# mkkellogg/GaussianSplats3D

Measured on AMD Instinct MI355X. Metric: Msplats/s sorted+rasterized at 1920x1080 SH-2, higher is better.
Workload: dtype int32 keys / f32 raster; 1 GPU; C3: garden.ply stand-in, SH2, 1920x1080; splats=5800000, sh_degree=2, width=1920, height=1080, cull=off (R=N), sort_precision_bits=16, streams=one (SURVEY.md 8d: sort -> draw on a single stream), parallelism=1 GPU, sort=full list (R = N)

## Files before the change

### gaussiansplats3d_amd/csrc/gs_internal.hpp

```cpp
#pragma once
#include <hip/hip_runtime.h>
#include <stdint.h>
#include <stdio.h>
#include <stdlib.h>
#include <string.h>
#include <new>
#include <utility>
#include <vector>

#include "../../include/gsplat_hip.h"
#include "draw_plan.hpp"

void gs_set_error(const char* fmt, ...);

#define GS_HIP(expr)                                                                              \
    do {                                                                                          \
        hipError_t _e = (expr);                                                                   \
        if (_e != hipSuccess) {                                                                   \
            gs_set_error("%s failed: %s (%s:%d)", #expr, hipGetErrorString(_e), __FILE__, __LINE__); \
            return GS_ERR_HIP;                                                                    \
        }                                                                                         \
    } while (0)

#define GS_REQUIRE(cond, msg)                                    \
// ... 162 lines not shown
    __host__ __device__ int32_t hi() const {
        int32_t v = key_max[0];
        for (uint32_t k = 1; k < SORT_SHARDS; k++) v = key_max[k] > v ? key_max[k] : v;
        return v;
    }
    uint32_t clamped;
    uint32_t kept;
};

struct gs_tree;
struct TreeGatherView {
    uint64_t tree_uid;
    uint32_t leaves, tree_splats;
    const uint32_t *leaf_offset, *leaf_count, *leaf_begin, *leaf_indexes, *totals;
};
void gs_tree_view(gs_tree* t, TreeGatherView* v);
int gs_tree_copy_plain(gs_tree* t, uint32_t* out_dev, hipStream_t st);
void gs_tree_forget_sorter(gs_tree* t, gs_sorter* s);

struct AssetDeviceImage {
    DevBuf bytes, table;
};

struct gs_sorter {
    gs_context* ctx = nullptr;
    AssetDeviceImage asset_dev;
    uint32_t max_count = 0, flags = 0, precision = 16, uploaded = 0;
    DevBuf cx, cy, cz, cw, scene_idx;
    DevBuf caos;
    DevBuf staging;
    DevBuf idx_in;
    DevBuf precomputed;
    DevBuf keys;
    DevBuf keyA, keyB, valA, valB;
    DevBuf sorted;
    DevBuf frame;
    uint32_t frame_index = 0;
    DevBuf scene_rows;
    DevBuf debug;
    RadixScratch radix;
    hipStream_t stream = nullptr;
    bool own_stream = false;
    hipEvent_t ev0 = nullptr, ev1 = nullptr;
    bool timed_sort = false;
    hipEvent_t ev_consumed = nullptr;
    bool consumer_pending = false;
    gs_mesh* bound_mesh = nullptr;
    gs_mesh* result_mesh = nullptr;
    const uint32_t* result_unmap = nullptr;
    uint32_t result_payload_max = 0;
    uint32_t gathered = 0;
    bool has_gathered = false;
    bool gathered_on_device = false;
    DevBuf gathered_dev;
    gs_tree* pending_tree = nullptr;
    bool pending_keep_zeroed = false;
    uint32_t centers_version = 0;
    DevBuf pay_in;
    DevBuf leaf_centers, leaf_pos;
    uint64_t leaf_cache_tree = 0;
    uint32_t leaf_cache_centers = 0, leaf_cache_layout = 0, leaf_cache_uploaded = 0;
    const void* leaf_cache_mesh = nullptr;
    uint32_t last_render = 0, last_sort = 0, last_passes = 0;
    bool last_identity = true;
    bool has_result = false;
    bool frustum_cull = false;
    bool visibility_cull = false;
    bool last_culled = false;
    const SortFrame* result_frame = nullptr;
    DevBuf keep_mask;
    DevBuf chunk_counts;
    DevBuf mask_copy;
    bool last_vis_culled = false;
    bool dev_distances = false;
    uint32_t dev_distances_count = 0;
    bool dev_distances_integer = false;
    hipEvent_t ev_handover = nullptr;
    std::vector<int32_t> extreme;
    bool extreme_ok = true;
    uint32_t extreme_version = 0;
    uint32_t clean_slot = 3;
    bool last_known_range = false;
    int32_t last_range_lo = 0, last_range_hi = 0;
    uint32_t last_pass0_slot = 0;
};

struct __attribute__((aligned(32))) SplatRec {
    float cx, cy, ax, ay;
    float bx, by;
    uint32_t c0, c1;
};
static_assert(sizeof(SplatRec) == 32, "SplatRec must be one 32-byte sector");

struct RenderFrame {
    uint32_t visible;
    uint32_t entries_lo;
    uint32_t entries_hi;
    uint32_t overflow;
    uint32_t entry_count;
    uint32_t tiles16_lo;
    uint32_t tiles16_hi;
    uint32_t pad;
};

struct ProjectParams {
    float view[16];
    float proj[16];
    float cam_pos[3];
    float focal_x, focal_y;
    float width, height;
    float splat_scale, kernel2d, max_splat_px, inv_focal_adj;
    uint32_t sh_degree;
    uint32_t sh_stored;
    uint32_t cov_half;
    uint32_t flags;
    uint32_t tiles_x, tiles_y;
    uint32_t row_begin, row_end;
// ... 170 lines not shown
```

### gaussiansplats3d_amd/csrc/sorter.hip

```cpp
#include <math.h>
#include <stdlib.h>

#include "extreme_set.hpp"
#include "radix.hpp"

__host__ __device__ static inline int32_t trunc_f64_i32(double v) {
    if (!(v > -2147483649.0 && v < 2147483648.0)) return INT32_MIN;
    return (int32_t)v;
}

constexpr uint32_t MODE_INT = 1, MODE_DYNAMIC = 2, MODE_PRECOMPUTED = 4;
#ifndef GS_KEY_GRID_MULT
#define GS_KEY_GRID_MULT 2
#endif

struct SceneRows {
    int32_t im[GS_MAX_SCENES][4];
    float fm[GS_MAX_SCENES][4];
};

struct KeyParams {
    const uint32_t *cx, *cy, *cz, *cw;
    const uint4* aos;
    const uint32_t* scene_idx;
// ... 641 lines not shown
        for (uint32_t u = 0; u < VC_UNROLL; u++) {
            const uint32_t i0 = wbase + u * VC_WAVE_SPAN + 4u * lane;
            if (i0 < end && (i0 & 31u) == 0u) {
                mask_copy[i0 >> 5] = cur.raw[u];
                if (cur.raw[u]) mask[i0 >> 5] = 0u;
            }
            uint32_t o = wave_out + first[u];
            const uint32_t pm[4] = {cur.M[u].x, cur.M[u].y, cur.M[u].z, cur.M[u].w};
#pragma unroll
            for (uint32_t c = 0; c < 4u; c++)
                if ((nibs[u] >> c) & 1u) {
                    keys_out[o] = K[u][c];
                    pay_out[o] = pm[c];
                    o++;
                }
        }
        cur = nxt;
    }
    mm.publish_wave(p.frame, blockIdx.x * 4u + wave);
}

struct DepthLoaderArgs {
    const int32_t* __restrict__ keys;
    const unsigned long long* __restrict__ keep;
    const uint32_t* __restrict__ idx;
    const uint32_t* __restrict__ map;
    SortFrame* frame;
    const uint32_t* n_dev;
    uint32_t sort_start, render_count, range;
    uint32_t last_splat;
    uint32_t count_clamps;
    int32_t lo;
    float range_map;
};
template <bool CULL, bool IDX>
struct DepthLoaderT : DepthLoaderArgs {
    __device__ __forceinline__ void prepare() {
        if (n_dev) render_count = *n_dev;
        const uint32_t l = threadIdx.x & (SORT_SHARDS - 1u);
        set_range(frame->key_min[l], frame->key_max[l]);
    }
    __device__ __forceinline__ void set_range(int32_t lo_shard, int32_t hi) {
        lo = lo_shard;
#pragma unroll
        for (int o = SORT_SHARDS / 2; o > 0; o >>= 1) {
            lo = min(lo, __shfl_xor(lo, o, 64));
            hi = max(hi, __shfl_xor(hi, o, 64));
        }
        set_known_range(lo, hi);
        lo = __builtin_amdgcn_readfirstlane(lo);
        range_map = __uint_as_float(__builtin_amdgcn_readfirstlane(__float_as_uint(range_map)));
    }
    __device__ __forceinline__ void set_known_range(int32_t key_lo, int32_t key_hi) {
        lo = key_lo;
        range_map = __fdiv_rn((float)(range - 1), __fsub_rn((float)key_hi, (float)key_lo));
    }
    __device__ __forceinline__ uint32_t count() const { return render_count - sort_start; }
    __device__ __forceinline__ uint32_t bucket(uint32_t i) const { return bucket_of<false>(keys[i]); }
    template <bool COUNT>
    __device__ __forceinline__ uint32_t bucket_of(int32_t depth) const {
        const int32_t diff = (int32_t)((uint32_t)depth - (uint32_t)lo);
        const float f = __fmul_rn((float)diff, range_map);
        const bool fits = f >= -2147483648.0f && f < 2147483648.0f;
        const int32_t b = fits ? (int32_t)f : 0;
        const bool under = b < 0, over = !under && (uint32_t)b >= range;
        if (COUNT && count_clamps && (under || over)) atomicAdd(&frame->clamped, 1u);
        return under ? 0u : (over ? range - 1u : (uint32_t)b);
    }
    __device__ __forceinline__ uint32_t key(uint32_t j) const { return (range - 1) - bucket(render_count - 1 - j); }
    __device__ __forceinline__ uint32_t payload(uint32_t i) const {
        const uint32_t o = IDX ? min(ld32(idx, i), last_splat) : i;
        return map ? ld32(map, o) : o;
    }
    __device__ __forceinline__ uint32_t val(uint32_t j) const { return payload(render_count - 1 - j); }
    struct Raw { int32_t depth; uint32_t payload; };
    static __device__ __forceinline__ int prof_slot(int) { return 0; }
    __device__ __forceinline__ uint32_t pre(uint32_t j) const {
        const uint32_t i = render_count - 1 - j;
        return IDX ? min(ld32(idx, i), last_splat) : i;
    }
    __device__ __forceinline__ Raw fetch(uint32_t j, uint32_t o) const {
        Raw r;
        r.depth = ld32(keys, render_count - 1 - j);
        r.payload = map ? ld32(map, o) : o;
        return r;
    }
    __device__ __forceinline__ void decode(const Raw& r, uint32_t& k, uint32_t& v) const {
        k = (range - 1) - bucket_of<false>(r.depth);
        v = r.payload;
    }
    typedef int32_t HRaw;
    __device__ __forceinline__ HRaw hist_fetch(uint32_t j) const { return ld32(keys, render_count - 1 - j); }
    __device__ __forceinline__ uint32_t hist_key(HRaw depth) const { return (range - 1) - bucket_of<true>(depth); }
    __device__ __forceinline__ bool valid(uint32_t j) const {
        if (!CULL) return true;
        const uint32_t i = render_count - 1 - j;
        return (ld32(keep, i >> 6) >> (i & 63u)) & 1ull;
    }
};
typedef DepthLoaderT<false, false> DepthLoader;

struct PackedLoader {
    const uint32_t* __restrict__ words;
    const uint32_t* __restrict__ n_dev;
    uint32_t n_host, val_bits;
    __device__ __forceinline__ void prepare() {}
    __device__ __forceinline__ uint32_t count() const { return n_dev ? *n_dev : n_host; }
    struct Raw { uint32_t w; };
    __device__ __forceinline__ uint32_t pre(uint32_t) const { return 0u; }
    __device__ __forceinline__ Raw fetch(uint32_t j, uint32_t) const { return Raw{ld32(words, j)}; }
    __device__ __forceinline__ void decode(const Raw& r, uint32_t& k, uint32_t& v) const {
        k = r.w >> val_bits;
        v = r.w & ((1u << val_bits) - 1u);
    }
    __device__ __forceinline__ bool valid(uint32_t) const { return true; }
    static __device__ __forceinline__ int prof_slot(int) { return 1; }
};

__global__ void k_copy_head(const uint32_t* __restrict__ idx, const uint32_t* __restrict__ map, uint32_t* __restrict__ out,
                            uint32_t n, uint32_t last_splat) {
    for (uint32_t i = blockIdx.x * blockDim.x + threadIdx.x; i < n; i += gridDim.x * blockDim.x) {
        const uint32_t o = idx ? min(idx[i], last_splat) : i;
        out[i] = map ? map[o] : o;
    }
}

__global__ void k_unmap(const uint32_t* __restrict__ in, const uint32_t* __restrict__ unmap, uint32_t* __restrict__ out,
                        uint32_t n, uint32_t last) {
    for (uint32_t i = blockIdx.x * blockDim.x + threadIdx.x; i < n; i += gridDim.x * blockDim.x) out[i] = unmap[min(in[i], last)];
}

constexpr uint32_t KEY_HIST_VECS = 3;
__global__ __launch_bounds__(HIST_THREADS) void k_depth_key_hist(KeyParams p, DepthLoader ld, int32_t key_lo, int32_t key_hi, int shift,
                                                                  uint32_t keep_slot, uint32_t* __restrict__ block_hist,
                                                                  uint32_t* __restrict__ group_rows) {
    __shared__ uint32_t s_hist[4][RADIX_BINS];
    const uint32_t tid = threadIdx.x, t = blockIdx.x * HIST_THREADS + tid;
    sort_begin(p, t, gridDim.x * HIST_THREADS, keep_slot);
    if (t < SORT_SHARDS) {
        p.frame->key_min[t] = key_lo;
        p.frame->key_max[t] = key_hi;
    }
    ld.set_known_range(key_lo, key_hi);
    for (uint32_t k = tid; k < 4u * RADIX_BINS; k += HIST_THREADS) (&s_hist[0][0])[k] = 0;
    __syncthreads();
    uint32_t* hist = s_hist[(tid >> 6) & 3u];
    const uint32_t R = p.render_count;
    const RadixChunk ch = radix_chunk(R);
    const uint32_t j0 = min(ch.tile_begin * (uint32_t)RADIX_TILE, R), j1 = min(ch.tile_end * (uint32_t)RADIX_TILE, R);
    const uint32_t p0 = R - j1, p1 = R - j0;
    auto count = [&](int32_t k) { atomicAdd(&hist[(ld.hist_key(k) >> shift) & 255u], 1u); };
    auto scalars = [&](uint32_t begin, uint32_t end) {
        for (uint32_t i = begin + tid; i < end; i += HIST_THREADS) {
            const int32_t k = static_key_int(p, p.cx[i], p.cy[i], p.cz[i]);
            p.keys_out[i] = k;
            count(k);
        }
    };
    const uint32_t a4 = (p0 + 3u) / 4u, b4 = p1 / 4u;
    if (a4 < b4) {
        scalars(p0, a4 * 4u);
        scalars(b4 * 4u, p1);
        const uint4* x4 = reinterpret_cast<const uint4*>(p.cx);
        const uint4* y4 = reinterpret_cast<const uint4*>(p.cy);
        const uint4* z4 = reinterpret_cast<const uint4*>(p.cz);
        int4* o4 = reinterpret_cast<int4*>(p.keys_out);
        for (uint32_t v0 = a4; v0 < b4; v0 += KEY_HIST_VECS * HIST_THREADS) {
            uint4 x[KEY_HIST_VECS], y[KEY_HIST_VECS], z[KEY_HIST_VECS];
#pragma unroll
            for (uint32_t k = 0; k < KEY_HIST_VECS; k++) {
                const uint32_t v = min(v0 + k * HIST_THREADS + tid, b4 - 1u);
                x[k] = x4[v]; y[k] = y4[v]; z[k] = z4[v];
            }
#pragma unroll
            for (uint32_t k = 0; k < KEY_HIST_VECS; k++) {
                const uint32_t v = v0 + k * HIST_THREADS + tid;
                const int4 key = static_key_int4(p, x[k], y[k], z[k]);
                if (v < b4) {
                    o4[v] = key;
                    count(key.x); count(key.y); count(key.z); count(key.w);
                }
            }
        }
    } else {
        scalars(p0, p1);
    }
    __syncthreads();
    if (tid >= RADIX_BINS || ch.tile_begin >= ch.tile_end) return;
    const uint32_t total = s_hist[0][tid] + s_hist[1][tid] + s_hist[2][tid] + s_hist[3][tid];
    block_hist[ch.id * RADIX_BINS + tid] = total;
    if (total) atomicAdd(&group_rows[(ch.id / RADIX_GROUP) * RADIX_BINS + tid], total);
}

__global__ void k_debug_buckets(DepthLoader ld, int32_t* out) {
    ld.prepare();
    for (uint32_t i = ld.sort_start + blockIdx.x * blockDim.x + threadIdx.x; i < ld.render_count;
         i += gridDim.x * blockDim.x)
        out[i] = (int32_t)ld.bucket(i);
}

struct Pass0Args {
    DepthLoaderArgs ld;
    uint32_t Rs, val_bits;
    int shift;
    bool pack, chunked, wide;
    void* kbuf0;
    uint32_t* vo;
    uint32_t* kept_out;
    int slot;
    bool skip_hist;
};
template <bool CULL, bool IDX>
static int depth_pass0(const RadixExec& ex, const Pass0Args& a) {
    typedef DepthLoaderT<CULL, IDX> L;
    const L d = {a.ld};
    L h = d;
    h.count_clamps = 1;
    if (a.pack && a.chunked) return radix_pass_chunk<L, L, true>(ex, h, a.shift, d, a.Rs, a.shift, a.slot, a.vo, a.val_bits, a.kept_out, a.skip_hist);
    if (a.pack) return radix_pass_ex<L, L, uint8_t, false, false, true>(ex, h, a.shift, d, a.Rs, a.shift, a.slot, (uint8_t*)nullptr, a.vo, nullptr, 0u, a.val_bits, a.kept_out, a.skip_hist);
    if (a.wide) return radix_pass_ex<L, L, uint32_t, true, false, false>(ex, h, a.shift, d, a.Rs, a.shift, a.slot, (uint32_t*)a.kbuf0, a.vo, nullptr, 0u, 0u, a.kept_out, a.skip_hist);
    return radix_pass_ex<L, L, uint16_t, true, false, false>(ex, h, a.shift, d, a.Rs, a.shift, a.slot, (uint16_t*)a.kbuf0, a.vo, nullptr, 0u, 0u, a.kept_out, a.skip_hist);
}

static inline uint32_t grid_for(uint32_t n, uint32_t per_block, uint32_t cap) {
    uint32_t g = (n + per_block - 1) / per_block;
    if (g < 1) g = 1;
    return g > cap ? cap : g;
}

#ifdef GS_RADIX_PROFILE
extern "C" int gs_debug_radix_prof(void* dst) {
    return (int)hipMemcpyFromSymbol(dst, HIP_SYMBOL(g_radix_prof), sizeof(g_radix_prof), 0, hipMemcpyDeviceToHost);
}
#endif

extern "C" {

int gs_sorter_create(gs_context* ctx, uint32_t max_splat_count, uint32_t flags, uint32_t precision_bits,
                     gs_sorter** out) {
    GS_REQUIRE(ctx && out, "ctx / out == NULL");
    *out = nullptr;
    GS_REQUIRE(max_splat_count > 0, "max_splat_count == 0");
    GS_REQUIRE((flags & ~(GS_SORT_INTEGER | GS_SORT_DYNAMIC)) == 0, "unknown sorter flags");
    const uint32_t max_bits = (flags & GS_SORT_INTEGER) ? 20u : 24u;
    GS_REQUIRE(precision_bits >= 10 && precision_bits <= max_bits, "precision outside the Viewer's clamp (10..20 int, 10..24 float)");
    ScopedDevice sd(ctx->device);
    gs_sorter* s = new (std::nothrow) gs_sorter();
    if (!s) return GS_ERR_NOMEM;
    s->ctx = ctx;
    s->max_count = max_splat_count;
    s->flags = flags;
    s->precision = precision_bits;
    const size_t n = max_splat_count, b4 = n * 4;
    int st = GS_OK;
    auto A = [&](DevBuf& b, size_t bytes) { if (st == GS_OK) st = b.alloc(bytes); };
    A(s->cx, b4 + 16); A(s->cy, b4 + 16); A(s->cz, b4 + 16); A(s->caos, n * 16);
    if (flags & GS_SORT_DYNAMIC) { A(s->cw, b4); A(s->scene_idx, b4); A(s->scene_rows, sizeof(SceneRows)); }
    A(s->keys, b4); A(s->keyA, b4); A(s->keyB, b4); A(s->valA, b4); A(s->valB, b4); A(s->sorted, b4);
    A(s->frame, 2 * sizeof(SortFrame));
    if (st == GS_OK) st = s->radix.init();
    if (st == GS_OK && (hipEventCreate(&s->ev0) != hipSuccess || hipEventCreate(&s->ev1) != hipSuccess ||
                        hipEventCreateWithFlags(&s->ev_consumed, hipEventDisableTiming) != hipSuccess ||
                        hipEventCreateWithFlags(&s->ev_handover, hipEventDisableTiming) != hipSuccess)) {
        gs_set_error("hipEventCreate failed");
        st = GS_ERR_HIP;
    }
    if (st == GS_OK) {
        SortFrame init[2];
        for (SortFrame& f : init) {
            for (uint32_t k = 0; k < SORT_SHARDS; k++) { f.key_min[k] = KEY_MIN_INIT; f.key_max[k] = KEY_MAX_INIT; }
            f.clamped = f.kept = 0;
        }
        if (hipMemcpy(s->frame.p, init, sizeof(init), hipMemcpyHostToDevice) != hipSuccess ||
            hipMemset(s->radix.digit_total.p, 0, sizeof(uint32_t) * RADIX_TOTAL_WORDS) != hipSuccess) {
            gs_set_error("initialising the sorter scratch failed");
            st = GS_ERR_HIP;
        }
    }
    if (st == GS_OK) {
        if (ctx->serial) {
            s->stream = ctx->stream;
        } else if (hipStreamCreateWithFlags(&s->stream, hipStreamNonBlocking) == hipSuccess) {
            s->own_stream = true;
        } else {
            gs_set_error("hipStreamCreate(sorter) failed");
            st = GS_ERR_HIP;
        }
    }
    if (st != GS_OK) {
        gs_sorter_destroy(s);
        return st;
// ... 22 lines not shown
    static const bool off = getenv("GSPLAT_NO_KNOWN_RANGE") != nullptr;
    return off;
}

static int sorter_update_extreme(gs_sorter* s, uint32_t from, uint32_t end, uint32_t old_uploaded, bool zero_fill) {
    if (s->flags != GS_SORT_INTEGER || known_range_off()) return GS_OK;
    const bool current = s->extreme_ok && s->extreme_version + 1u == s->centers_version;
    const bool append = from >= old_uploaded;
    if (append && !current) {
        s->extreme_ok = false;
        return GS_OK;
    }
    const uint32_t first = append ? old_uploaded : 0u, last = end > old_uploaded ? end : old_uploaded;
    std::vector<int32_t> rows, out;
    try {
        if (zero_fill && append) rows.assign(4, 0);
        else rows.resize((size_t)(last - first) * 4);
    } catch (const std::bad_alloc&) {
        s->extreme_ok = false;
        return GS_OK;
    }
    if (!(zero_fill && append) && last > first) {
        GS_HIP(hipMemcpyAsync(rows.data(), s->caos.as<uint4>() + first, (size_t)(last - first) * 16, hipMemcpyDeviceToHost, s->stream));
        GS_HIP(hipStreamSynchronize(s->stream));
    }
    const bool prior = append && !s->extreme.empty();
    s->extreme_ok = gs_extreme_set(prior ? s->extreme.data() : nullptr, prior ? s->extreme.size() / 4 : 0, rows.data(), rows.size() / 4,
                                   GS_EXTREME_CAP, out);
    s->extreme.swap(out);
    s->extreme_version = s->centers_version;
    return GS_OK;
}

int gs_sorter_upload_centers(gs_sorter* s, uint32_t from, uint32_t count, const void* centers_aos4,
                             const uint32_t* scene_indexes) {
    GS_REQUIRE(s && centers_aos4, "sorter / centers == NULL");
    GS_REQUIRE((uint64_t)from + count <= s->max_count, "range exceeds max_splat_count");
    GS_REQUIRE(!(s->flags & GS_SORT_DYNAMIC) || scene_indexes, "dynamic sorter needs scene_indexes");
    if (count == 0) return GS_OK;
    ScopedDevice sd(s->ctx->device);
    GS_HIP(hipMemcpyAsync(s->caos.as<uint4>() + from, centers_aos4, (size_t)count * 16, hipMemcpyHostToDevice, s->stream));
    return gs_sorter_commit_centers(s, from, count, scene_indexes);
}

}

int gs_sorter_commit_centers(gs_sorter* s, uint32_t from, uint32_t count, const uint32_t* scene_indexes) {
    hipStream_t st = s->stream;
    uint4* aos = s->caos.as<uint4>() + from;
    hipLaunchKernelGGL(k_aos4_to_soa, dim3(grid_for(count, 256, 4096)), dim3(256), 0, st, aos, count,
                       from, s->cx.as<uint32_t>(), s->cy.as<uint32_t>(), s->cz.as<uint32_t>(),
                       (s->flags & GS_SORT_DYNAMIC) ? s->cw.as<uint32_t>() : nullptr);
    GS_HIP(hipGetLastError());
    if (s->flags & GS_SORT_DYNAMIC)
        GS_HIP(hipMemcpyAsync(s->scene_idx.as<uint32_t>() + from, scene_indexes, (size_t)count * 4, hipMemcpyHostToDevice, st));
    GS_HIP(hipStreamSynchronize(st));
    const uint32_t old_uploaded = s->uploaded;
    if (from + count > s->uploaded) s->uploaded = from + count;
    s->centers_version++;
    GS_TRY(sorter_update_extreme(s, from, from + count, old_uploaded, false));
    sorter_tell_mesh(s);
    return GS_OK;
}

extern "C" {

int gs_sorter_set_uploaded_count(gs_sorter* s, uint32_t count) {
    GS_REQUIRE(s != nullptr, "sorter == NULL");
    GS_REQUIRE(count <= s->max_count, "count exceeds max_splat_count");
    if (count <= s->uploaded) return GS_OK;
    ScopedDevice sd(s->ctx->device);
    hipStream_t st = s->stream;
    const size_t from = s->uploaded, n = count - s->uploaded;
    GS_HIP(hipMemsetAsync(s->caos.as<uint4>() + from, 0, n * 16, st));
    DevBuf* planes[] = {&s->cx, &s->cy, &s->cz, &s->cw, &s->scene_idx};
    for (DevBuf* b : planes)
        if (b->p) GS_HIP(hipMemsetAsync(b->as<uint32_t>() + from, 0, n * 4, st));
    GS_HIP(hipStreamSynchronize(st));
    s->uploaded = count;
    s->centers_version++;
    GS_TRY(sorter_update_extreme(s, (uint32_t)from, count, (uint32_t)from, true));
    sorter_tell_mesh(s);
    return GS_OK;
}

static int sorter_collect_stats(gs_sorter* s, gs_sort_stats* stats) {
    SortFrame f;
    GS_HIP(hipMemcpyAsync(&f, s->frame.as<SortFrame>() + s->frame_index, sizeof(f), hipMemcpyDeviceToHost, s->stream));
    GS_HIP(hipStreamSynchronize(s->stream));
    float ms = 0.f;
    if (s->timed_sort) GS_HIP(hipEventElapsedTime(&ms, s->ev0, s->ev1));
    int32_t key_lo = f.lo(), key_hi = f.hi();
    if (s->last_sort == 0) {
        key_lo = KEY_MIN_INIT;
        key_hi = KEY_MAX_INIT;
        f.clamped = 0;
    }
    stats->device_ms = ms;
    stats->key_min = key_lo;
    stats->key_max = key_hi;
    stats->clamped = f.clamped;
    stats->passes = s->last_passes;
    stats->result_count = s->last_culled ? f.kept : s->last_render;
    return f.clamped ? GS_WARN_KEY_CLAMPED : GS_OK;
}

struct SortSwitches {
    bool tree_no_fuse;
    const char* vis_front;
    bool no_pack;
    bool no_chunk;
    bool no_known_range;
};
static SortSwitches sort_switches() {
    static const bool tree_no_fuse = getenv("GSPLAT_TREE_NO_FUSE") != nullptr;
    static const char* vis_front = getenv("GSPLAT_VIS_FRONT");
    static const bool no_pack = getenv("GSPLAT_NO_SORT_PACK") != nullptr;
    static const bool no_chunk = getenv("GSPLAT_NO_SORT_CHUNK") != nullptr;
    return {tree_no_fuse, vis_front, no_pack, no_chunk, known_range_off()};
}

static bool sorter_mesh_alive(const gs_context* ctx, const gs_mesh* m) {
    for (const gs_mesh* l : ctx->live_meshes)
        if (l == m) return m != nullptr;
    return false;
}

struct ChunkGrid { uint32_t grid, len; };
static ChunkGrid chunk_grid(const gs_context* ctx, uint32_t R, uint32_t unit) {
    const uint32_t units = (R + unit - 1u) / unit;
    const uint32_t grid = units < (uint32_t)ctx->cu_count * 2u ? units : (uint32_t)ctx->cu_count * 2u;
    return {grid, ((units + grid - 1u) / grid) * unit};
}

struct SortPlan {
    const float* mvp;
    const uint32_t* indexes_to_sort;
    bool device_list;
    const void* precomputed;
    const float* transforms;
    const uint32_t* list_count_dev;
    uint32_t R, Rs, sort_start;
    bool pre_device, dynamic;
    bool vis_cull;
    bool cull;
    const uint32_t *map, *unmap;
    uint32_t last_splat;
    uint32_t max_payload, val_bits;
    SortSwitches sw;
    const uint32_t* idx_dev;
    bool fused_tree;
    bool vec4;
    bool vis_front;
    bool known_range;
    int32_t range_lo, range_hi;
    uint32_t pass0_slot;
};

struct Pass0Shape { bool pack, chunked; uint32_t grid; };
static Pass0Shape pass0_shape(const gs_sorter* s, const SortPlan& pl) {
    Pass0Shape sh;
    sh.chunked = !pl.sw.no_chunk && pl.val_bits <= 24u && radix_chunk_grid_for(pl.Rs) != 0u;
    sh.pack = s->precision > 8u && !pl.sw.no_pack && (s->precision - 8u) + pl.val_bits <= 32u;
    sh.grid = (sh.pack && sh.chunked) ? radix_chunk_grid_for(pl.Rs) : radix_grid_for(pl.Rs);
    return sh;
}

static bool sort_known_range(const gs_sorter* s, const SortPlan& pl, const KeyParams& kp, int32_t& lo_out, int32_t& hi_out) {
    if (pl.sw.no_known_range || kp.mode != MODE_INT || pl.idx_dev || pl.device_list || pl.fused_tree || pl.vis_cull || pl.cull ||
        pl.list_count_dev || pl.sort_start != 0u || pl.R != s->uploaded || pl.R == 0u)
        return false;
    if (!s->extreme_ok || s->extreme_version != s->centers_version || s->extreme.empty()) return false;
    const int32_t* c = s->extreme.data();
    const size_t n = s->extreme.size() / 4;
    const int64_t a0 = kp.im0, a1 = kp.im1, a2 = kp.im2;
    const int64_t small = (int64_t)1 << 29;
    __int128 lo, hi;
    if (a0 >= -small && a0 <= small && a1 >= -small && a1 <= small && a2 >= -small && a2 <= small) {
        int64_t l = INT64_MAX, h = INT64_MIN;
        for (size_t i = 0; i < n; i++) {
            const int64_t v = a0 * c[4 * i] + a1 * c[4 * i + 1] + a2 * c[4 * i + 2];
            l = v < l ? v : l;
            h = v > h ? v : h;
        }
        lo = l; hi = h;
    } else {
        lo = hi = (__int128)a0 * c[0] + (__int128)a1 * c[1] + (__int128)a2 * c[2];
        for (size_t i = 1; i < n; i++) {
// ... 199 lines not shown
        if (lazy) derive();
        else hipLaunchKernelGGL(k_mask_count, dim3(wg.grid), dim3(VC_THREADS), 0, st, kp, mask, wg.len, counts);
        if (pl.map) hipLaunchKernelGGL(k_cull_front<true>, dim3(wg.grid), dim3(VC_THREADS), 0, st, kp, mask, s->mask_copy.as<uint32_t>(),
                                       counts, wg.len, pl.map, s->pay_in.as<uint32_t>(), lazy ? DERIVE_SUBS : 1u);
        else hipLaunchKernelGGL(k_cull_front<false>, dim3(wg.grid), dim3(VC_THREADS), 0, st, kp, mask, s->mask_copy.as<uint32_t>(),
                                counts, wg.len, pl.map, s->pay_in.as<uint32_t>(), 1u);
    } else {
        const ChunkGrid cg = chunk_grid(ctx, R, VC_SPAN);
        if (!s->pending_tree) s->has_gathered = false;
        GS_TRY(s->chunk_counts.ensure((size_t)std::max(lazy ? dg.grid * DERIVE_SUBS : 0u, cg.grid) * 4));
        counts = s->chunk_counts.as<uint32_t>();
        if (lazy) derive();
        hipLaunchKernelGGL(k_minmax_count, dim3(cg.grid), dim3(VC_THREADS), 0, st, kp, mask, cg.len, counts);
        hipLaunchKernelGGL(k_mask_compact, dim3(cg.grid), dim3(VC_THREADS), 0, st, mask, s->mask_copy.as<uint32_t>(), counts, R, cg.len,
                           s->idx_in.as<uint32_t>(), kp.frame);
    }
    if (R >= mesh->vis_orig_count && (!lazy || mesh->vis_orig_tail_zero)) mesh->vis_orig_dirty = false;
    pl.idx_dev = s->idx_in.as<uint32_t>();
    kp.idx_in = pl.idx_dev;
    kp.count_dev = &kp.frame->kept;
    kp.ext_minmax = 1u;
    if (!pl.vis_front) hipLaunchKernelGGL(k_depth_key<false>, dim3(grid_for(pl.Rs, 256 * 4, (uint32_t)ctx->cu_count * 2)), dim3(256), 0, st, kp);
    return GS_OK;
}

static int launch_front_end(gs_sorter* s, SortPlan& pl, KeyParams& kp) {
    gs_context* ctx = s->ctx;
    hipStream_t st = s->stream;
    const uint32_t cus = (uint32_t)ctx->cu_count;
    pl.vec4 = (kp.mode == MODE_INT) && !pl.idx_dev;
    pl.known_range = sort_known_range(s, pl, kp, pl.range_lo, pl.range_hi);
    pl.pass0_slot = pl.known_range ? s->clean_slot : 0u;
    s->clean_slot = pl.pass0_slot == 3u ? 0u : 3u;
    if (pl.known_range) {
        DepthLoaderArgs hl = {};
        hl.keys = s->keys.as<int32_t>(); hl.frame = kp.frame; hl.sort_start = 0u; hl.render_count = pl.R; hl.range = 1u << s->precision;
        hl.last_splat = kp.last_splat; hl.count_clamps = 1u;
        hipLaunchKernelGGL(k_depth_key_hist, dim3(pass0_shape(s, pl).grid), dim3(HIST_THREADS), 0, st, kp, DepthLoader{hl}, pl.range_lo,
                           pl.range_hi, 0, pl.pass0_slot, s->radix.block_hist.as<uint32_t>(),
                           s->radix.digit_total.as<uint32_t>() + pl.pass0_slot * RADIX_SLOT_WORDS);
    } else if (pl.fused_tree) {
        GS_TRY(launch_tree_front(s, pl, kp));
    } else if (pl.vis_cull) {
        GS_TRY(launch_vis_cull_front(s, pl, kp));
    } else if (pl.cull) {
        if (pl.vec4) hipLaunchKernelGGL(k_depth_key_cull<true>, dim3(grid_for(pl.Rs, 256 * 16, cus * 2)), dim3(256), 0, st, kp);
        else hipLaunchKernelGGL(k_depth_key_cull<false>, dim3(grid_for(pl.Rs, 256 * 4, cus * 4)), dim3(256), 0, st, kp);
    } else if (pl.vec4) {
        hipLaunchKernelGGL(k_depth_key<true>, dim3(grid_for(pl.Rs, 256 * 16, cus * GS_KEY_GRID_MULT)), dim3(256), 0, st, kp);
    } else {
        hipLaunchKernelGGL(k_depth_key<false>, dim3(grid_for(pl.Rs, 256 * 4, cus * 2)), dim3(256), 0, st, kp);
    }
    GS_HIP(hipGetLastError());
    return GS_OK;
}

static int run_radix_passes(gs_sorter* s, const SortPlan& pl, const KeyParams& kp) {
    const RadixExec ex = {s->stream, &s->radix, s->ctx->lds_atomic_lane_order};
    const uint32_t Rs = pl.Rs, val_bits = pl.val_bits;
    const bool own_payloads = pl.fused_tree || pl.vis_front;
    DepthLoaderArgs dl = {};
    dl.keys = s->keys.as<int32_t>();
    dl.keep = pl.cull ? kp.keep : nullptr;
    dl.idx = own_payloads ? s->pay_in.as<uint32_t>() : pl.idx_dev;
    dl.map = own_payloads ? nullptr : pl.map;
    dl.frame = kp.frame;
    dl.sort_start = pl.sort_start;
    dl.render_count = pl.R;
    dl.range = 1u << s->precision;
    dl.last_splat = own_payloads ? pl.max_payload : kp.last_splat;
    dl.n_dev = pl.vis_cull ? &kp.frame->kept : pl.list_count_dev;
    const uint32_t passes = (s->precision + 7) / 8;
    uint32_t* out_tail = s->sorted.as<uint32_t>() + pl.sort_start;
    void* kbuf[2] = {s->keyA.p, s->keyB.p};
    uint32_t* vbuf[2] = {s->valA.as<uint32_t>(), s->valB.as<uint32_t>()};
    const bool chunked = pass0_shape(s, pl).chunked;
    const bool wide = s->precision > 16;
    const uint32_t* n_dev = (pl.cull || pl.vis_cull || pl.list_count_dev) ? &kp.frame->kept : nullptr;
    bool in_packed = false;
    for (uint32_t p = 0; p < passes; p++) {
        const bool last = (p + 1 == passes);
        const int left = (int)s->precision - 8 * (int)(p + 1);
        const bool pack = !last && !pl.sw.no_pack && (uint32_t)left + val_bits <= 32u;
        const int shift = in_packed ? 0 : 8 * (int)p;
        uint32_t* vo = last ? out_tail : vbuf[p & 1];
        if (p == 0) {
            Pass0Args a = {};
            a.ld = dl; a.Rs = Rs; a.val_bits = val_bits; a.shift = shift;
            a.pack = pack; a.chunked = chunked; a.wide = wide; a.kbuf0 = kbuf[0]; a.vo = vo;
            a.kept_out = pl.cull ? &kp.frame->kept : nullptr;
            a.slot = (int)pl.pass0_slot;
            a.skip_hist = pl.known_range;
            const bool has_idx = dl.idx != nullptr;
            if (pl.cull && has_idx) GS_TRY((depth_pass0<true, true>(ex, a)));
            else if (pl.cull) GS_TRY((depth_pass0<true, false>(ex, a)));
            else if (has_idx) GS_TRY((depth_pass0<false, true>(ex, a)));
            else GS_TRY((depth_pass0<false, false>(ex, a)));
        } else if (in_packed) {
            PackedLoader pk = {vbuf[(p - 1) & 1], n_dev, Rs, val_bits};
            ArrayLoader<uint32_t> ph = {vbuf[(p - 1) & 1], nullptr, n_dev, Rs};
            if (chunked && last) GS_TRY((radix_pass_chunk<ArrayLoader<uint32_t>, PackedLoader, false>(ex, ph, (int)val_bits, pk, Rs, 0, (int)p, vo, 0u)));
            else if (chunked) GS_TRY((radix_pass_chunk<ArrayLoader<uint32_t>, PackedLoader, true>(ex, ph, (int)val_bits, pk, Rs, 0, (int)p, vo, val_bits)));
            else if (last) GS_TRY((radix_pass_ex<ArrayLoader<uint32_t>, PackedLoader, uint8_t, false, false, false>(ex, ph, (int)val_bits, pk, Rs, 0, (int)p, (uint8_t*)nullptr, vo, nullptr, 0u, 0u)));
            else GS_TRY((radix_pass_ex<ArrayLoader<uint32_t>, PackedLoader, uint8_t, false, false, true>(ex, ph, (int)val_bits, pk, Rs, 0, (int)p, (uint8_t*)nullptr, vo, nullptr, 0u, val_bits)));
        } else if (wide) {
            ArrayLoader<uint32_t> al = {(const uint32_t*)kbuf[(p - 1) & 1], vbuf[(p - 1) & 1], n_dev, Rs};
            if (last) GS_TRY((radix_pass<ArrayLoader<uint32_t>, uint32_t, false>(ex, al, al, Rs, shift, (int)p, (uint32_t*)nullptr, vo)));
            else if (pack) GS_TRY((radix_pass_ex<ArrayLoader<uint32_t>, ArrayLoader<uint32_t>, uint8_t, false, false, true>(ex, al, shift, al, Rs, shift, (int)p, (uint8_t*)nullptr, vo, nullptr, 0u, val_bits)));
            else GS_TRY((radix_pass<ArrayLoader<uint32_t>, uint32_t, true>(ex, al, al, Rs, shift, (int)p, (uint32_t*)kbuf[p & 1], vo)));
        } else {
            ArrayLoader<uint16_t> al = {(const uint16_t*)kbuf[(p - 1) & 1], vbuf[(p - 1) & 1], n_dev, Rs};
            if (last) GS_TRY((radix_pass<ArrayLoader<uint16_t>, uint16_t, false>(ex, al, al, Rs, shift, (int)p, (uint16_t*)nullptr, vo)));
            else GS_TRY((radix_pass<ArrayLoader<uint16_t>, uint16_t, true>(ex, al, al, Rs, shift, (int)p, (uint16_t*)kbuf[p & 1], vo)));
        }
        in_packed = in_packed || pack;
    }
    return GS_OK;
}

static int sort_finish(gs_sorter* s, const SortPlan& pl, const KeyParams& kp, uint32_t passes, uint32_t* sorted_out, gs_sort_stats* stats) {
    hipStream_t st = s->stream;
    if (pl.sort_start > 0) {
        hipLaunchKernelGGL(k_copy_head, dim3(grid_for(pl.sort_start, 1024, 2048)), dim3(256), 0, st, pl.idx_dev, pl.map,
                           s->sorted.as<uint32_t>(), pl.sort_start, s->uploaded - 1u);
    }
    GS_HIP(hipGetLastError());
    if (s->timed_sort || st != s->ctx->stream) GS_HIP(hipEventRecord(s->ev1, st));
    s->last_render = pl.R;
    s->last_sort = pl.Rs;
    s->last_passes = passes;
    s->last_known_range = pl.known_range;
    s->last_range_lo = pl.known_range ? pl.range_lo : 0;
    s->last_range_hi = pl.known_range ? pl.range_hi : 0;
    s->last_pass0_slot = pl.pass0_slot;
    s->last_identity = (pl.idx_dev == nullptr);
    s->last_culled = (pl.cull || pl.vis_cull || pl.list_count_dev) && pl.Rs > 0;
    s->last_vis_culled = pl.vis_cull && pl.Rs > 0;
    s->result_frame = kp.frame;
    s->result_mesh = pl.map ? s->bound_mesh : nullptr;
    s->result_unmap = pl.unmap;
    s->result_payload_max = pl.max_payload;
    s->has_result = true;

    uint32_t out_count = pl.R;
    if (sorted_out && s->last_culled) {
        SortFrame f;
        GS_HIP(hipMemcpyAsync(&f, kp.frame, sizeof(f), hipMemcpyDeviceToHost, st));
        GS_HIP(hipStreamSynchronize(st));
        out_count = f.kept;
    }
    if (sorted_out && out_count) {
        const void* src = s->sorted.p;
        if (pl.unmap) {
            GS_TRY(s->debug.ensure((size_t)s->max_count * 4));
            hipLaunchKernelGGL(k_unmap, dim3(grid_for(out_count, 1024, 2048)), dim3(256), 0, st, s->sorted.as<uint32_t>(), pl.unmap,
                               s->debug.as<uint32_t>(), out_count, s->result_payload_max);
            GS_HIP(hipGetLastError());
            src = s->debug.p;
        }
        GS_HIP(hipMemcpyAsync(sorted_out, src, (size_t)out_count * 4, hipMemcpyDeviceToHost, st));
        GS_HIP(hipStreamSynchronize(st));
    }
    return stats ? sorter_collect_stats(s, stats) : GS_OK;
}

static int sorter_sort(gs_sorter* s, const float* mvp, const uint32_t* indexes_to_sort, bool device_list, uint32_t sort_count,
                       uint32_t render_count, const void* precomputed, const float* transforms, uint32_t* sorted_out,
// ... 49 lines not shown
    if (s->bound_mesh != m && sorter_mesh_alive(s->ctx, s->bound_mesh)) s->bound_mesh->derive_orig_mask = false;
    s->bound_mesh = m;
    sorter_tell_mesh(s);
    return GS_OK;
}

int gs_sorter_set_frustum_cull(gs_sorter* s, int enable) {
    GS_REQUIRE(s != nullptr, "sorter == NULL");
    GS_REQUIRE(!enable || !(s->flags & GS_SORT_DYNAMIC), "the per-splat frustum cull is not available to a dynamic-mode sorter");
    s->frustum_cull = enable != 0;
    return GS_OK;
}

int gs_sorter_set_visibility_cull(gs_sorter* s, int enable) {
    GS_REQUIRE(s != nullptr, "sorter == NULL");
    GS_REQUIRE(!enable || !(s->flags & GS_SORT_DYNAMIC), "the visibility cull is not available to a dynamic-mode sorter");
    s->visibility_cull = enable != 0;
    sorter_tell_mesh(s);
    return GS_OK;
}

int gs_sorter_last_stats(gs_sorter* s, gs_sort_stats* stats) {
    GS_REQUIRE(s && stats, "sorter / stats == NULL");
    GS_REQUIRE(s->has_result, "no sort has run");
    ScopedDevice sd(s->ctx->device);
    return sorter_collect_stats(s, stats);
}

int gs_sorter_debug_read(gs_sorter* s, int what, void* dst, uint32_t count) {
    GS_REQUIRE(s && dst, "sorter / dst == NULL");
    GS_REQUIRE(s->has_result, "no sort has run");
    if (what == 4) {
        const bool valid = s->extreme_ok && s->extreme_version == s->centers_version;
        const int32_t w[6] = {s->last_known_range ? 1 : 0, valid ? (int32_t)(s->extreme.size() / 4) : 0, s->last_range_lo, s->last_range_hi,
                              valid ? 1 : 0, (int32_t)s->last_pass0_slot};
        GS_REQUIRE(count <= 6u, "selector 4 holds 6 words");
        memcpy(dst, w, (size_t)count * 4);
        return GS_OK;
    }
    GS_REQUIRE(count <= s->last_render, "count exceeds the last render_count");
    ScopedDevice sd(s->ctx->device);
    hipStream_t st = s->stream;
    const void* src = nullptr;
    if (what == 0) src = s->keys.p;
    else if (what == 2) {
        src = s->sorted.p;
        if (sorter_mesh_alive(s->ctx, s->result_mesh) && s->result_unmap && count) {
            GS_TRY(s->debug.ensure((size_t)s->max_count * 4));
            hipLaunchKernelGGL(k_unmap, dim3(grid_for(count, 1024, 2048)), dim3(256), 0, st, s->sorted.as<uint32_t>(),
                               s->result_unmap, s->debug.as<uint32_t>(), count, s->result_payload_max);
            GS_HIP(hipGetLastError());
            src = s->debug.p;
        }
    }
    else if (what == 1) {
        GS_TRY(s->debug.ensure((size_t)s->max_count * 4));
        DepthLoaderArgs dl = {};
        dl.keys = s->keys.as<int32_t>();
        dl.frame = s->frame.as<SortFrame>() + s->frame_index;
        dl.sort_start = s->last_render - s->last_sort;
        dl.render_count = s->last_render;
        dl.range = 1u << s->precision;
        GS_HIP(hipMemsetAsync(s->debug.p, 0, (size_t)s->last_render * 4, st));
        if (s->last_sort)
            hipLaunchKernelGGL(k_debug_buckets, dim3(grid_for(s->last_sort, 1024, 2048)), dim3(256), 0, st, DepthLoader{dl}, s->debug.as<int32_t>());
        GS_HIP(hipGetLastError());
        src = s->debug.p;
    } else if (what == 3) {
        GS_REQUIRE(s->last_culled, "the last sort did not cull");
        if (s->last_vis_culled) {
            GS_REQUIRE((size_t)count * 4 <= s->mask_copy.bytes, "count exceeds the mask length");
            src = s->mask_copy.p;
        } else {
            GS_REQUIRE((size_t)count * 4 <= s->keep_mask.bytes, "count exceeds the mask length");
            src = s->keep_mask.p;
        }
// ... 10 lines not shown
```

Before: 25820 Msplats/s.

## Emit 16-bit pre-bucketed depth keys in fused key/histogram pass when range known

When the depth range is known and precision is at most 16 bits, the fused key+histogram kernel now writes already-bucketed 16-bit keys to a new keys16 buffer instead of 32-bit raw depths. Pass 0 of the radix sort then reads these narrow keys directly and skips the bucket recomputation. This halves key write and read traffic for the first pass. The 32-bit keys buffer is marked stale and lazily regenerated by a new kernel only when debug reads or center uploads need it, which adds bookkeeping and an extra buffer.

```diff
diff --git a/gaussiansplats3d_amd/csrc/gs_internal.hpp b/gaussiansplats3d_amd/csrc/gs_internal.hpp
--- a/gaussiansplats3d_amd/csrc/gs_internal.hpp
+++ b/gaussiansplats3d_amd/csrc/gs_internal.hpp
@@ -218,6 +218,7 @@
     DevBuf idx_in;
     DevBuf precomputed;
     DevBuf keys;
+    DevBuf keys16;
     DevBuf keyA, keyB, valA, valB;
     DevBuf sorted;
     DevBuf frame;
@@ -269,6 +270,10 @@
     bool last_known_range = false;
     int32_t last_range_lo = 0, last_range_hi = 0;
     uint32_t last_pass0_slot = 0;
+    bool last_narrow = false;
+    bool keys_stale = false;
+    int32_t stale_im[3] = {0, 0, 0};
+    uint32_t stale_count = 0;
 };
 
 struct __attribute__((aligned(32))) SplatRec {
diff --git a/gaussiansplats3d_amd/csrc/sorter.hip b/gaussiansplats3d_amd/csrc/sorter.hip
--- a/gaussiansplats3d_amd/csrc/sorter.hip
+++ b/gaussiansplats3d_amd/csrc/sorter.hip
@@ -697,10 +697,12 @@
     uint32_t count_clamps;
     int32_t lo;
     float range_map;
+    const uint16_t* __restrict__ keys16;
 };
-template <bool CULL, bool IDX>
+template <bool CULL, bool IDX, bool NARROW = false>
 struct DepthLoaderT : DepthLoaderArgs {
     __device__ __forceinline__ void prepare() {
+        if (NARROW) return;
         if (n_dev) render_count = *n_dev;
         const uint32_t l = threadIdx.x & (SORT_SHARDS - 1u);
         set_range(frame->key_min[l], frame->key_max[l]);
@@ -746,17 +748,19 @@
     }
     __device__ __forceinline__ Raw fetch(uint32_t j, uint32_t o) const {
         Raw r;
-        r.depth = ld32(keys, render_count - 1 - j);
+        r.depth = NARROW ? (int32_t)ld32(keys16, render_count - 1 - j) : ld32(keys, render_count - 1 - j);
         r.payload = map ? ld32(map, o) : o;
         return r;
     }
     __device__ __forceinline__ void decode(const Raw& r, uint32_t& k, uint32_t& v) const {
-        k = (range - 1) - bucket_of<false>(r.depth);
+        k = NARROW ? (uint32_t)r.depth : (range - 1) - bucket_of<false>(r.depth);
         v = r.payload;
     }
     typedef int32_t HRaw;
-    __device__ __forceinline__ HRaw hist_fetch(uint32_t j) const { return ld32(keys, render_count - 1 - j); }
-    __device__ __forceinline__ uint32_t hist_key(HRaw depth) const { return (range - 1) - bucket_of<true>(depth); }
+    __device__ __forceinline__ HRaw hist_fetch(uint32_t j) const {
+        return NARROW ? (int32_t)ld32(keys16, render_count - 1 - j) : ld32(keys, render_count - 1 - j);
+    }
+    __device__ __forceinline__ uint32_t hist_key(HRaw depth) const { return NARROW ? (uint32_t)depth : (range - 1) - bucket_of<true>(depth); }
     __device__ __forceinline__ bool valid(uint32_t j) const {
         if (!CULL) return true;
         const uint32_t i = render_count - 1 - j;
@@ -796,9 +800,13 @@
 }
 
 constexpr uint32_t KEY_HIST_VECS = 3;
+#ifndef GS_KEY_HIST_PAIR
+#define GS_KEY_HIST_PAIR 1
+#endif
+template <bool NARROW>
 __global__ __launch_bounds__(HIST_THREADS) void k_depth_key_hist(KeyParams p, DepthLoader ld, int32_t key_lo, int32_t key_hi, int shift,
                                                                   uint32_t keep_slot, uint32_t* __restrict__ block_hist,
-                                                                  uint32_t* __restrict__ group_rows) {
+                                                                  uint32_t* __restrict__ group_rows, uint16_t* __restrict__ keys16) {
     __shared__ uint32_t s_hist[4][RADIX_BINS];
     const uint32_t tid = threadIdx.x, t = blockIdx.x * HIST_THREADS + tid;
     sort_begin(p, t, gridDim.x * HIST_THREADS, keep_slot);
@@ -814,36 +822,58 @@
     const RadixChunk ch = radix_chunk(R);
     const uint32_t j0 = min(ch.tile_begin * (uint32_t)RADIX_TILE, R), j1 = min(ch.tile_end * (uint32_t)RADIX_TILE, R);
     const uint32_t p0 = R - j1, p1 = R - j0;
-    auto count = [&](int32_t k) { atomicAdd(&hist[(ld.hist_key(k) >> shift) & 255u], 1u); };
+    auto count = [&](int32_t k) {
+        const uint32_t r = ld.hist_key(k);
+        atomicAdd(&hist[(r >> shift) & 255u], 1u);
+        return r;
+    };
     auto scalars = [&](uint32_t begin, uint32_t end) {
         for (uint32_t i = begin + tid; i < end; i += HIST_THREADS) {
             const int32_t k = static_key_int(p, p.cx[i], p.cy[i], p.cz[i]);
-            p.keys_out[i] = k;
-            count(k);
+            const uint32_t r = count(k);
+            if (NARROW) keys16[i] = (uint16_t)r;
+            else p.keys_out[i] = k;
         }
     };
-    const uint32_t a4 = (p0 + 3u) / 4u, b4 = p1 / 4u;
-    if (a4 < b4) {
-        scalars(p0, a4 * 4u);
-        scalars(b4 * 4u, p1);
+    constexpr uint32_t VPU = (NARROW && GS_KEY_HIST_PAIR) ? 2u : 1u, UPOS = 4u * VPU;
+    constexpr uint32_t UNITS = VPU == 2u ? (uint32_t)(GS_KEY_HIST_PAIR ? GS_KEY_HIST_PAIR : 1) : KEY_HIST_VECS;
+    const uint32_t a = (p0 + UPOS - 1u) / UPOS, b = p1 / UPOS;
+    if (a < b) {
+        scalars(p0, a * UPOS);
+        scalars(b * UPOS, p1);
         const uint4* x4 = reinterpret_cast<const uint4*>(p.cx);
         const uint4* y4 = reinterpret_cast<const uint4*>(p.cy);
         const uint4* z4 = reinterpret_cast<const uint4*>(p.cz);
         int4* o4 = reinterpret_cast<int4*>(p.keys_out);
-        for (uint32_t v0 = a4; v0 < b4; v0 += KEY_HIST_VECS * HIST_THREADS) {
-            uint4 x[KEY_HIST_VECS], y[KEY_HIST_VECS], z[KEY_HIST_VECS];
-#pragma unroll
-            for (uint32_t k = 0; k < KEY_HIST_VECS; k++) {
-                const uint32_t v = min(v0 + k * HIST_THREADS + tid, b4 - 1u);
-                x[k] = x4[v]; y[k] = y4[v]; z[k] = z4[v];
+        for (uint32_t u0 = a; u0 < b; u0 += UNITS * HIST_THREADS) {
+            uint4 x[UNITS][VPU], y[UNITS][VPU], z[UNITS][VPU];
+#pragma unroll
+            for (uint32_t k = 0; k < UNITS; k++) {
+                const uint32_t u = min(u0 + k * HIST_THREADS + tid, b - 1u);
+#pragma unroll
+                for (uint32_t q = 0; q < VPU; q++) { x[k][q] = x4[u * VPU + q]; y[k][q] = y4[u * VPU + q]; z[k][q] = z4[u * VPU + q]; }
             }
 #pragma unroll
-            for (uint32_t k = 0; k < KEY_HIST_VECS; k++) {
-                const uint32_t v = v0 + k * HIST_THREADS + tid;
-                const int4 key = static_key_int4(p, x[k], y[k], z[k]);
-                if (v < b4) {
-                    o4[v] = key;
-                    count(key.x); count(key.y); count(key.z); count(key.w);
+            for (uint32_t k = 0; k < UNITS; k++) {
+                const uint32_t u = u0 + k * HIST_THREADS + tid;
+                int4 key[VPU];
+#pragma unroll
+                for (uint32_t q = 0; q < VPU; q++) key[q] = static_key_int4(p, x[k][q], y[k][q], z[k][q]);
+                if (u < b) {
+                    if constexpr (NARROW) {
+                        uint32_t w[2u * VPU];
+#pragma unroll
+                        for (uint32_t q = 0; q < VPU; q++) {
+                            const uint32_t r0 = count(key[q].x), r1 = count(key[q].y), r2 = count(key[q].z), r3 = count(key[q].w);
+                            w[2u * q] = r0 | (r1 << 16);
+                            w[2u * q + 1u] = r2 | (r3 << 16);
+                        }
+                        if constexpr (VPU == 2u) reinterpret_cast<uint4*>(keys16)[u] = make_uint4(w[0], w[1], w[2], w[3]);
+                        else reinterpret_cast<uint2*>(keys16)[u] = make_uint2(w[0], w[1]);
+                    } else {
+                        o4[u] = key[0];
+                        count(key[0].x); count(key[0].y); count(key[0].z); count(key[0].w);
+                    }
                 }
             }
         }
@@ -862,6 +892,11 @@
     for (uint32_t i = ld.sort_start + blockIdx.x * blockDim.x + threadIdx.x; i < ld.render_count;
          i += gridDim.x * blockDim.x)
         out[i] = (int32_t)ld.bucket(i);
+}
+
+__global__ __launch_bounds__(256) void k_debug_rekey(KeyParams p, uint32_t n) {
+    for (uint32_t i = blockIdx.x * blockDim.x + threadIdx.x; i < n; i += gridDim.x * blockDim.x)
+        p.keys_out[i] = static_key_int(p, p.cx[i], p.cy[i], p.cz[i]);
 }
 
 struct Pass0Args {
@@ -875,15 +910,16 @@
     int slot;
     bool skip_hist;
 };
-template <bool CULL, bool IDX>
+template <bool CULL, bool IDX, bool NARROW = false>
 static int depth_pass0(const RadixExec& ex, const Pass0Args& a) {
-    typedef DepthLoaderT<CULL, IDX> L;
+    typedef DepthLoaderT<CULL, IDX, NARROW> L;
     const L d = {a.ld};
     L h = d;
     h.count_clamps = 1;
     if (a.pack && a.chunked) return radix_pass_chunk<L, L, true>(ex, h, a.shift, d, a.Rs, a.shift, a.slot, a.vo, a.val_bits, a.kept_out, a.skip_hist);
     if (a.pack) return radix_pass_ex<L, L, uint8_t, false, false, true>(ex, h, a.shift, d, a.Rs, a.shift, a.slot, (uint8_t*)nullptr, a.vo, nullptr, 0u, a.val_bits, a.kept_out, a.skip_hist);
-    if (a.wide) return radix_pass_ex<L, L, uint32_t, true, false, false>(ex, h, a.shift, d, a.Rs, a.shift, a.slot, (uint32_t*)a.kbuf0, a.vo, nullptr, 0u, 0u, a.kept_out, a.skip_hist);
+    if constexpr (!NARROW)
+        if (a.wide) return radix_pass_ex<L, L, uint32_t, true, false, false>(ex, h, a.shift, d, a.Rs, a.shift, a.slot, (uint32_t*)a.kbuf0, a.vo, nullptr, 0u, 0u, a.kept_out, a.skip_hist);
     return radix_pass_ex<L, L, uint16_t, true, false, false>(ex, h, a.shift, d, a.Rs, a.shift, a.slot, (uint16_t*)a.kbuf0, a.vo, nullptr, 0u, 0u, a.kept_out, a.skip_hist);
 }
 
@@ -922,6 +958,7 @@
     A(s->cx, b4 + 16); A(s->cy, b4 + 16); A(s->cz, b4 + 16); A(s->caos, n * 16);
     if (flags & GS_SORT_DYNAMIC) { A(s->cw, b4); A(s->scene_idx, b4); A(s->scene_rows, sizeof(SceneRows)); }
     A(s->keys, b4); A(s->keyA, b4); A(s->keyB, b4); A(s->valA, b4); A(s->valB, b4); A(s->sorted, b4);
+    A(s->keys16, n * 2 + 16);
     A(s->frame, 2 * sizeof(SortFrame));
     if (st == GS_OK) st = s->radix.init();
     if (st == GS_OK && (hipEventCreate(&s->ev0) != hipSuccess || hipEventCreate(&s->ev1) != hipSuccess ||
@@ -1010,6 +1047,19 @@
     return GS_OK;
 }
 
+static int sorter_refresh_keys(gs_sorter* s) {
+    if (!s->keys_stale) return GS_OK;
+    KeyParams kp = {};
+    kp.cx = s->cx.as<uint32_t>(); kp.cy = s->cy.as<uint32_t>(); kp.cz = s->cz.as<uint32_t>();
+    kp.keys_out = s->keys.as<int32_t>();
+    kp.mode = MODE_INT;
+    kp.im0 = s->stale_im[0]; kp.im1 = s->stale_im[1]; kp.im2 = s->stale_im[2];
+    hipLaunchKernelGGL(k_debug_rekey, dim3(grid_for(s->stale_count, 1024, 2048)), dim3(256), 0, s->stream, kp, s->stale_count);
+    GS_HIP(hipGetLastError());
+    s->keys_stale = false;
+    return GS_OK;
+}
+
 int gs_sorter_upload_centers(gs_sorter* s, uint32_t from, uint32_t count, const void* centers_aos4,
                              const uint32_t* scene_indexes) {
     GS_REQUIRE(s && centers_aos4, "sorter / centers == NULL");
@@ -1017,6 +1067,7 @@
     GS_REQUIRE(!(s->flags & GS_SORT_DYNAMIC) || scene_indexes, "dynamic sorter needs scene_indexes");
     if (count == 0) return GS_OK;
     ScopedDevice sd(s->ctx->device);
+    GS_TRY(sorter_refresh_keys(s));
     GS_HIP(hipMemcpyAsync(s->caos.as<uint4>() + from, centers_aos4, (size_t)count * 16, hipMemcpyHostToDevice, s->stream));
     return gs_sorter_commit_centers(s, from, count, scene_indexes);
 }
@@ -1025,6 +1076,7 @@
 
 int gs_sorter_commit_centers(gs_sorter* s, uint32_t from, uint32_t count, const uint32_t* scene_indexes) {
     hipStream_t st = s->stream;
+    GS_TRY(sorter_refresh_keys(s));
     uint4* aos = s->caos.as<uint4>() + from;
     hipLaunchKernelGGL(k_aos4_to_soa, dim3(grid_for(count, 256, 4096)), dim3(256), 0, st, aos, count,
                        from, s->cx.as<uint32_t>(), s->cy.as<uint32_t>(), s->cz.as<uint32_t>(),
@@ -1089,13 +1141,15 @@
     bool no_pack;
     bool no_chunk;
     bool no_known_range;
+    bool no_narrow_keys;
 };
 static SortSwitches sort_switches() {
     static const bool tree_no_fuse = getenv("GSPLAT_TREE_NO_FUSE") != nullptr;
     static const char* vis_front = getenv("GSPLAT_VIS_FRONT");
     static const bool no_pack = getenv("GSPLAT_NO_SORT_PACK") != nullptr;
     static const bool no_chunk = getenv("GSPLAT_NO_SORT_CHUNK") != nullptr;
-    return {tree_no_fuse, vis_front, no_pack, no_chunk, known_range_off()};
+    static const bool no_narrow_keys = getenv("GSPLAT_NO_NARROW_KEYS") != nullptr;
+    return {tree_no_fuse, vis_front, no_pack, no_chunk, known_range_off(), no_narrow_keys};
 }
 
 static bool sorter_mesh_alive(const gs_context* ctx, const gs_mesh* m) {
@@ -1132,6 +1186,7 @@
     bool vis_front;
     bool known_range;
     int32_t range_lo, range_hi;
+    bool narrow;
     uint32_t pass0_slot;
 };
 
@@ -1397,13 +1452,19 @@
     pl.known_range = sort_known_range(s, pl, kp, pl.range_lo, pl.range_hi);
     pl.pass0_slot = pl.known_range ? s->clean_slot : 0u;
     s->clean_slot = pl.pass0_slot == 3u ? 0u : 3u;
+    pl.narrow = pl.known_range && s->precision <= 16u && !pl.sw.no_narrow_keys;
     if (pl.known_range) {
         DepthLoaderArgs hl = {};
         hl.keys = s->keys.as<int32_t>(); hl.frame = kp.frame; hl.sort_start = 0u; hl.render_count = pl.R; hl.range = 1u << s->precision;
         hl.last_splat = kp.last_splat; hl.count_clamps = 1u;
-        hipLaunchKernelGGL(k_depth_key_hist, dim3(pass0_shape(s, pl).grid), dim3(HIST_THREADS), 0, st, kp, DepthLoader{hl}, pl.range_lo,
-                           pl.range_hi, 0, pl.pass0_slot, s->radix.block_hist.as<uint32_t>(),
-                           s->radix.digit_total.as<uint32_t>() + pl.pass0_slot * RADIX_SLOT_WORDS);
+        const dim3 grid(pass0_shape(s, pl).grid);
+        uint32_t* group_rows = s->radix.digit_total.as<uint32_t>() + pl.pass0_slot * RADIX_SLOT_WORDS;
+        if (pl.narrow)
+            hipLaunchKernelGGL(k_depth_key_hist<true>, grid, dim3(HIST_THREADS), 0, st, kp, DepthLoader{hl}, pl.range_lo, pl.range_hi, 0,
+                               pl.pass0_slot, s->radix.block_hist.as<uint32_t>(), group_rows, s->keys16.as<uint16_t>());
+        else
+            hipLaunchKernelGGL(k_depth_key_hist<false>, grid, dim3(HIST_THREADS), 0, st, kp, DepthLoader{hl}, pl.range_lo, pl.range_hi, 0,
+                               pl.pass0_slot, s->radix.block_hist.as<uint32_t>(), group_rows, (uint16_t*)nullptr);
     } else if (pl.fused_tree) {
         GS_TRY(launch_tree_front(s, pl, kp));
     } else if (pl.vis_cull) {
@@ -1426,6 +1487,7 @@
     const bool own_payloads = pl.fused_tree || pl.vis_front;
     DepthLoaderArgs dl = {};
     dl.keys = s->keys.as<int32_t>();
+    dl.keys16 = s->keys16.as<uint16_t>();
     dl.keep = pl.cull ? kp.keep : nullptr;
     dl.idx = own_payloads ? s->pay_in.as<uint32_t>() : pl.idx_dev;
     dl.map = own_payloads ? nullptr : pl.map;
@@ -1457,7 +1519,8 @@
             a.slot = (int)pl.pass0_slot;
             a.skip_hist = pl.known_range;
             const bool has_idx = dl.idx != nullptr;
-            if (pl.cull && has_idx) GS_TRY((depth_pass0<true, true>(ex, a)));
+            if (pl.narrow) GS_TRY((depth_pass0<false, false, true>(ex, a)));
+            else if (pl.cull && has_idx) GS_TRY((depth_pass0<true, true>(ex, a)));
             else if (pl.cull) GS_TRY((depth_pass0<true, false>(ex, a)));
             else if (has_idx) GS_TRY((depth_pass0<false, true>(ex, a)));
             else GS_TRY((depth_pass0<false, false>(ex, a)));
@@ -1498,6 +1561,12 @@
     s->last_range_lo = pl.known_range ? pl.range_lo : 0;
     s->last_range_hi = pl.known_range ? pl.range_hi : 0;
     s->last_pass0_slot = pl.pass0_slot;
+    s->last_narrow = pl.narrow;
+    if (pl.Rs > 0) {
+        s->keys_stale = pl.narrow;
+        s->stale_im[0] = kp.im0; s->stale_im[1] = kp.im1; s->stale_im[2] = kp.im2;
+        s->stale_count = pl.R;
+    }
     s->last_identity = (pl.idx_dev == nullptr);
     s->last_culled = (pl.cull || pl.vis_cull || pl.list_count_dev) && pl.Rs > 0;
     s->last_vis_culled = pl.vis_cull && pl.Rs > 0;
@@ -1613,9 +1682,9 @@
     GS_REQUIRE(s->has_result, "no sort has run");
     if (what == 4) {
         const bool valid = s->extreme_ok && s->extreme_version == s->centers_version;
-        const int32_t w[6] = {s->last_known_range ? 1 : 0, valid ? (int32_t)(s->extreme.size() / 4) : 0, s->last_range_lo, s->last_range_hi,
-                              valid ? 1 : 0, (int32_t)s->last_pass0_slot};
-        GS_REQUIRE(count <= 6u, "selector 4 holds 6 words");
+        const int32_t w[7] = {s->last_known_range ? 1 : 0, valid ? (int32_t)(s->extreme.size() / 4) : 0, s->last_range_lo, s->last_range_hi,
+                              valid ? 1 : 0, (int32_t)s->last_pass0_slot, s->last_narrow ? 1 : 0};
+        GS_REQUIRE(count <= 7u, "selector 4 holds 7 words");
         memcpy(dst, w, (size_t)count * 4);
         return GS_OK;
     }
@@ -1623,6 +1692,7 @@
     ScopedDevice sd(s->ctx->device);
     hipStream_t st = s->stream;
     const void* src = nullptr;
+    if (what == 0 || what == 1) GS_TRY(sorter_refresh_keys(s));
     if (what == 0) src = s->keys.p;
     else if (what == 2) {
         src = s->sorted.p;
```

After: 26170 Msplats/s, median of 6. +1.4%, better.
